# gmongaras/Stable-Diffusion-3-From-Scratch

Measured on AMD Instinct MI355X. Metric: train images/sec MMDiT-B 256^2 bf16, higher is better.
Workload: dtype bf16

## Files before the change

stable-diffusion-3-from-scratch_amd/csrc/rowops.hip:

```cpp
#include "qk_rows.h"
#include "fp8_quant.h"
#include "../../include/mmdit_hip_hd128.h"
#include "../../include/mmdit_hip_mxpad.h"

namespace {

constexpr float LN_EPS = 1e-5f;

__device__ __forceinline__ float bf16_round(float x) { return __builtin_bit_cast(float, pack_bf2(x, 0.f) << 16); }

template <int NITX, typename TO, typename TA, bool RES, bool MX = false, bool PAD = false>
__device__ __forceinline__ void ln_mod_fwd_body(int block, const float* __restrict__ x, const float* __restrict__ scale, const float* __restrict__ shift,
                                                int64_t ld_mod, int rows, int d, int rpb, TO* __restrict__ out,
                                                float* __restrict__ mean_o, float* __restrict__ rstd_o,
                                                const TA* __restrict__ acc, const float* __restrict__ gate, int64_t ld_gate, float* __restrict__ xo,
                                                unsigned char* __restrict__ mx_scales) {
  constexpr int NIT = NITX < 0 ? -NITX : NITX;
  constexpr bool EXACT = NITX < 0;
  const int lane = threadIdx.x & 63, row = block * 4 + (threadIdx.x >> 6);
  if (row >= rows) return;
  const int nch = d >> 2;
  const int b = row / rpb;
  const float* xr = x + (int64_t)row * d;
  float v[NIT][4];
  float s = 0.f;
#pragma unroll
  for (int it = 0; it < NIT; it++) {
    int ch = lane + 64 * it;
    if (EXACT || ch < nch) {
      ld4(xr + ch * 4, v[it]);
      if constexpr (RES) {
        float av[4], g[4];
        ld4(acc + (int64_t)row * d + ch * 4, av);
        ld4(gate + (int64_t)b * ld_gate + ch * 4, g);
#pragma unroll
        for (int e = 0; e < 4; e++) v[it][e] = v[it][e] + g[e] * av[e];
        __builtin_nontemporal_store(f32x4{v[it][0], v[it][1], v[it][2], v[it][3]}, (f32x4*)(xo + (int64_t)row * d + ch * 4));
      }
      s += v[it][0] + v[it][1] + v[it][2] + v[it][3];
    }
    else { v[it][0] = v[it][1] = v[it][2] = v[it][3] = 0.f; }
  }
  const float mean = wave_sum(s) / d;
  float q = 0.f;
#pragma unroll
  for (int it = 0; it < NIT; it++) {
    int ch = lane + 64 * it;
    if (EXACT || ch < nch) {
#pragma unroll
      for (int e = 0; e < 4; e++) { float c = v[it][e] - mean; q += c * c; }
    }
  }
  const float rstd = rsqrtf(wave_sum(q) / d + LN_EPS);
  if (lane == 0) { mean_o[row] = mean; rstd_o[row] = rstd; }
  const float* sc = scale + (int64_t)b * ld_mod;
  const float* sh = shift + (int64_t)b * ld_mod;
  TO* orow = out + (int64_t)row * d;
  const int ldo = PAD ? d + 64 : d;
  if constexpr (PAD) {
    if (lane < 4) *(uint4*)((unsigned char*)out + (int64_t)row * ldo + d + lane * 16) = make_uint4(0u, 0u, 0u, 0u);
    if (lane < 2) mx_scales[mx_scale_index(row, (d >> 5) + lane, rows)] = 0;
  }
#pragma unroll
  for (int it = 0; it < NIT; it++) {
    int ch = lane + 64 * it;
    if (EXACT || ch < nch) {
      float a[4], h[4], o[4];
      ld4(sc + ch * 4, a); ld4(sh + ch * 4, h);
#pragma unroll
      for (int e = 0; e < 4; e++) o[e] = (v[it][e] - mean) * rstd * (1.f + a[e]) + h[e];
      if constexpr (MX) {
#pragma unroll
        for (int e = 0; e < 4; e++) o[e] = bf16_round(o[e]);
        float amax = fmaxf(fmaxf(fabsf(o[0]), fabsf(o[1])), fmaxf(fabsf(o[2]), fabsf(o[3])));
        amax = fmaxf(amax, __shfl_xor(amax, 1, 64));
        amax = fmaxf(amax, __shfl_xor(amax, 2, 64));
        amax = fmaxf(amax, __shfl_xor(amax, 4, 64));
        float inv;
        const int ex = mx_exponent(amax, inv);
        *(unsigned*)((unsigned char*)out + (int64_t)row * ldo + ch * 4) = mx_pack4(o, inv);
        if ((lane & 7) == 0) mx_scales[mx_scale_index(row, ch >> 3, rows)] = (unsigned char)(ex + 127);
      } else {
        st4(orow + ch * 4, o);
      }
    }
  }
}

struct LnFwdProb {
  const float* x; const float* scale; const float* shift; int64_t ld_mod; int rows, rpb; void* out; float* mean; float* rstd;
  const void* acc; const float* gate; int64_t ld_gate; float* xo; unsigned char* mx_scales;
};
template <int NIT, typename TO, typename TA, bool RES, bool MX = false, bool PAD = false>
__global__ __launch_bounds__(256) void ln_mod_fwd_kernel(LnFwdProb p0, LnFwdProb p1, int nblk0, int d) {
  const bool first = (int)blockIdx.x < nblk0;
  const LnFwdProb& p = first ? p0 : p1;
  ln_mod_fwd_body<NIT, TO, TA, RES, MX, PAD>(first ? (int)blockIdx.x : (int)blockIdx.x - nblk0, p.x, p.scale, p.shift, p.ld_mod, p.rows, d, p.rpb, (TO*)p.out, p.mean, p.rstd,
                                        (const TA*)p.acc, p.gate, p.ld_gate, p.xo, p.mx_scales);
}

template <typename TA>
__global__ __launch_bounds__(256) void gate_residual_fwd_kernel(const float* __restrict__ x, const TA* __restrict__ acc, const float* __restrict__ gate, int64_t ld_gate,
                                                                int rows, int d, int rpb, float* __restrict__ out) {
  const int nch = d >> 2;
  for (int64_t i = (int64_t)blockIdx.x * 256 + threadIdx.x; i < (int64_t)rows * nch; i += (int64_t)gridDim.x * 256) {
    const int row = (int)(i / nch), ch = (int)(i - (int64_t)row * nch);
    float xv[4], av[4], g[4];
    ld4(x + (int64_t)row * d + ch * 4, xv);
    ld4(acc + (int64_t)row * d + ch * 4, av);
    ld4(gate + (int64_t)(row / rpb) * ld_gate + ch * 4, g);
#pragma unroll
    for (int e = 0; e < 4; e++) xv[e] = xv[e] + g[e] * av[e];
    st4(out + (int64_t)row * d + ch * 4, xv);
  }
}

#ifndef MMDIT_LN_BWD_RCH
#define MMDIT_LN_BWD_RCH 16
#endif
constexpr int LN_BWD_RCH = MMDIT_LN_BWD_RCH;
template <int NITX, typename TG, typename TA, bool GATED>
__device__ __forceinline__ void ln_mod_bwd_body(int block, const TG* __restrict__ dout, const float* __restrict__ x, const float* __restrict__ mean_i,
                                                const float* __restrict__ rstd_i, const float* __restrict__ scale, int64_t ld_mod,
                                                const float* __restrict__ dres, int d, int rpb, int nchunk,
                                                float* __restrict__ dx, float* __restrict__ dscale, float* __restrict__ dshift, int64_t ld_dmod,
                                                const TA* __restrict__ acc, const float* __restrict__ gate, int64_t ld_gate, TA* __restrict__ dacc,
                                                float* __restrict__ dgate, int64_t ld_dgate, float* __restrict__ dbias, int64_t ld_dbias, int rch = LN_BWD_RCH) {
  constexpr int NIT = NITX < 0 ? -NITX : NITX;
  constexpr bool EXACT = NITX < 0;
  const int lane = threadIdx.x & 63, wave = threadIdx.x >> 6;
  const int b = block / nchunk, chunk = block % nchunk;
  const int nch = d >> 2;
  const float* sc = scale + (int64_t)b * ld_mod;
  __shared__ float s_a1[NIT * 256], s_gt[GATED ? NIT * 256 : 4];
  for (int c = threadIdx.x; c < NIT * 256; c += 256) {
    s_a1[c] = c < d ? sc[c] + 1.f : 0.f;
    if constexpr (GATED) s_gt[c] = c < d ? gate[(int64_t)b * ld_gate + c] : 0.f;
  }
  __syncthreads();
  float ds[NIT][4], dh[NIT][4];
  float sg[GATED ? NIT : 1][4], sb[GATED ? NIT : 1][4];
#pragma unroll
  for (int it = 0; it < NIT; it++) {
#pragma unroll
    for (int e = 0; e < 4; e++) { ds[it][e] = 0.f; dh[it][e] = 0.f; }
    if constexpr (GATED) {
#pragma unroll
      for (int e = 0; e < 4; e++) { sg[it][e] = 0.f; sb[it][e] = 0.f; }
    }
  }
  const int rend = min(rpb, (chunk + 1) * rch);
  for (int rl = chunk * rch + wave; rl < rend; rl += 4) {
    const int64_t row = (int64_t)b * rpb + rl;
    const float mean = mean_i[row], rstd = rstd_i[row];
    float g[NIT][4], xh[NIT][4];
    float c1 = 0.f, c2 = 0.f;
    asm volatile("" ::: "memory");
#pragma unroll
    for (int it = 0; it < NIT; it++) {
      int ch = lane + 64 * it;
      if (EXACT || ch < nch) {
        float dy[4], xv[4], a1[4];
        ld4_nt(dout + row * d + ch * 4, dy);
        ld4_nt(x + row * d + ch * 4, xv);
        ld4(s_a1 + ch * 4, a1);
#pragma unroll
        for (int e = 0; e < 4; e++) {
          xh[it][e] = (xv[e] - mean) * rstd;
          g[it][e] = dy[e] * a1[e];
          c1 += g[it][e]; c2 += g[it][e] * xh[it][e];
          ds[it][e] += dy[e] * xh[it][e]; dh[it][e] += dy[e];
        }
      }
    }
    c1 = wave_sum(c1) / d; c2 = wave_sum(c2) / d;
#pragma unroll
    for (int it = 0; it < NIT; it++) {
      int ch = lane + 64 * it;
      if (EXACT || ch < nch) {
        float o[4];
        if (dres) ld4(dres + row * d + ch * 4, o); else { o[0] = o[1] = o[2] = o[3] = 0.f; }
#pragma unroll
        for (int e = 0; e < 4; e++) o[e] += rstd * (g[it][e] - c1 - xh[it][e] * c2);
        st4(dx + row * d + ch * 4, o);
        if constexpr (GATED) {
          float av[4], da[4], gt[4];
          ld4_nt(acc + row * d + ch * 4, av);
          ld4(s_gt + ch * 4, gt);
#pragma unroll
          for (int e = 0; e < 4; e++) { da[e] = o[e] * gt[e]; sg[it][e] += o[e] * av[e]; sb[it][e] += da[e]; }
          st4(dacc + row * d + ch * 4, da);
        }
      }
    }
  }
  if constexpr (NIT <= 6) {
    __shared__ float red[4][NIT * 256];
    auto flush = [&](const float (&v)[NIT][4], float* dst) {
#pragma unroll
      for (int it = 0; it < NIT; it++)
#pragma unroll
        for (int e = 0; e < 4; e++) red[wave][(it * 64 + lane) * 4 + e] = v[it][e];
      __syncthreads();
      for (int c = threadIdx.x; c < d; c += 256) atomicAdd(dst + c, red[0][c] + red[1][c] + red[2][c] + red[3][c]);
      __syncthreads();
    };
    flush(ds, dscale + (int64_t)b * ld_dmod);
    flush(dh, dshift + (int64_t)b * ld_dmod);
    if constexpr (GATED) {
      flush(sg, dgate + (int64_t)b * ld_dgate);
      if (dbias) flush(sb, dbias + (int64_t)b * ld_dbias);
    }
  } else {
    auto flush = [&](const float (&v)[NIT][4], float* dst) {
#pragma unroll
      for (int it = 0; it < NIT; it++) {
        int ch = lane + 64 * it;
        if (EXACT || ch < nch) {
#pragma unroll
          for (int e = 0; e < 4; e++) atomicAdd(dst + ch * 4 + e, v[it][e]);
        }
      }
    };
    flush(ds, dscale + (int64_t)b * ld_dmod);
    flush(dh, dshift + (int64_t)b * ld_dmod);
    if constexpr (GATED) {
      flush(sg, dgate + (int64_t)b * ld_dgate);
      if (dbias) flush(sb, dbias + (int64_t)b * ld_dbias);
    }
  }
}

struct LnBwdProb {
  const void* dout; const float* x; const float* mean; const float* rstd; const float* scale; int64_t ld_mod; const float* dres; int rpb, nchunk;
  float* dx; float* dscale; float* dshift; int64_t ld_dmod;
  const void* acc; const float* gate; int64_t ld_gate; void* dacc; float* dgate; int64_t ld_dgate; float* dbias; int64_t ld_dbias;
};
template <int NIT, typename TG, typename TA, bool GATED>
__global__ __launch_bounds__(256) void ln_mod_bwd_kernel(LnBwdProb p0, LnBwdProb p1, int nblk0, int d, int rch) {
  const bool first = (int)blockIdx.x < nblk0;
  const LnBwdProb& p = first ? p0 : p1;
  ln_mod_bwd_body<NIT, TG, TA, GATED>(first ? (int)blockIdx.x : (int)blockIdx.x - nblk0, (const TG*)p.dout, p.x, p.mean, p.rstd, p.scale, p.ld_mod, p.dres, d, p.rpb, p.nchunk,
                                      p.dx, p.dscale, p.dshift, p.ld_dmod, (const TA*)p.acc, p.gate, p.ld_gate, (TA*)p.dacc, p.dgate, p.ld_dgate, p.dbias, p.ld_dbias, rch);
}

template <int NITX, typename TI, typename TO>
__global__ __launch_bounds__(256) void text_rms_fwd_kernel(const TI* __restrict__ x, const float* __restrict__ w, const float* __restrict__ sp,
                                                           int rows, int cnt, int tokens, int off, int d, TO* __restrict__ out) {
  constexpr int NIT = NITX < 0 ? -NITX : NITX;
  constexpr bool EXACT = NITX < 0;
  const int lane = threadIdx.x & 63, m = blockIdx.x * 4 + (threadIdx.x >> 6);
// ... 593 lines not shown
    float* dst = which == 0 ? dgate + (int64_t)b * ld_dgate : (dbias ? dbias + (int64_t)b * ld_dbias : nullptr);
    if (!dst) break;
#pragma unroll
    for (int e = 0; e < 8; e++) sbuf[ty * 256 + tx * 8 + e] = which == 0 ? sgate[e] : sb[e];
    __syncthreads();
    if (col < d) {
      float s = 0.f;
#pragma unroll
      for (int r = 0; r < 8; r++) s += sbuf[r * 256 + threadIdx.x];
      atomicAdd(dst + col, s);
    }
    __syncthreads();
  }
}

template <typename T>
__global__ __launch_bounds__(256) void colsum_kernel(const T* __restrict__ x, int rows, int cols, int64_t ld, float* __restrict__ out, int rch) {
  __shared__ float sbuf[1024];
  const int tx = threadIdx.x & 127, ty = threadIdx.x >> 7;
  const int c = blockIdx.x * 1024 + tx * 8;
  float s[8];
#pragma unroll
  for (int e = 0; e < 8; e++) s[e] = 0.f;
  if (c < cols) {
    const int rend = min(rows, (int)(blockIdx.y + 1) * rch);
#pragma unroll 4
    for (int r = blockIdx.y * rch + ty; r < rend; r += 2) {
      float v[8];
      ld8(x + r * ld + c, v);
#pragma unroll
      for (int e = 0; e < 8; e++) s[e] += v[e];
    }
  }
  colsum_flush(s, sbuf, out, c, cols);
}

template <typename TG, typename TO>
__global__ __launch_bounds__(256) void silu_bwd_kernel(const TG* __restrict__ dy, const float* __restrict__ pre, TO* __restrict__ dpre, int rpg, int cols, float* __restrict__ dbias) {
  __shared__ float sb[4][64];
  const int cl = threadIdx.x & 63, rl = threadIdx.x >> 6;
  const int c = blockIdx.x * 64 + cl;
  const int r0 = blockIdx.y * rpg;
  float s = 0.f;
  if (c < cols) {
#pragma unroll 4
    for (int r = r0 + rl; r < r0 + rpg; r += 4) {
      const int64_t i = (int64_t)r * cols + c;
      const float p = pre[i], sig = sigmoid_f(p);
      const float g = io<TG>::ld(dy + i) * sig * (1.f + p * (1.f - sig));
      io<TO>::st(dpre + i, g);
      s += g;
    }
  }
  sb[rl][cl] = s;
  __syncthreads();
  if (rl == 0 && c < cols && dbias) dbias[(int64_t)blockIdx.y * cols + c] += sb[0][cl] + sb[1][cl] + sb[2][cl] + sb[3][cl];
}

template <typename TI, typename TO>
__global__ void cast_kernel(const TI* __restrict__ src, TO* __restrict__ dst, int64_t n) {
  const int64_t n8 = n >> 3;
  for (int64_t i = (int64_t)blockIdx.x * blockDim.x + threadIdx.x; i < n8; i += (int64_t)gridDim.x * blockDim.x) {
    float v[8];
    ld8(src + i * 8, v);
    st8(dst + i * 8, v);
  }
  if (blockIdx.x == 0 && threadIdx.x < (n & 7)) io<TO>::st(dst + n8 * 8 + threadIdx.x, io<TI>::ld(src + n8 * 8 + threadIdx.x));
}

template <typename TI, typename TO, bool TO_TOKENS>
__global__ void patch_kernel(const TI* __restrict__ src, TO* __restrict__ dst, int batch, int ch, int H, int W) {
  const int W2 = W >> 1, H2 = H >> 1;
  const int64_t total = (int64_t)batch * ch * H * W2;
  for (int64_t g = (int64_t)blockIdx.x * blockDim.x + threadIdx.x; g < total; g += (int64_t)gridDim.x * blockDim.x) {
    const int j = (int)(g % W2); int64_t r = g / W2;
    const int y = (int)(r % H); r /= H;
    const int c = (int)(r % ch); const int64_t b = r / ch;
    const int64_t img_off = ((b * ch + c) * H + y) * W + 2 * j;
    const int64_t tok_off = ((b * H2 + (y >> 1)) * W2 + j) * (int64_t)(ch * 4) + c * 4 + (y & 1) * 2;
    if (TO_TOKENS) { io<TO>::st(dst + tok_off, io<TI>::ld(src + img_off)); io<TO>::st(dst + tok_off + 1, io<TI>::ld(src + img_off + 1)); }
    else { io<TO>::st(dst + img_off, io<TI>::ld(src + tok_off)); io<TO>::st(dst + img_off + 1, io<TI>::ld(src + tok_off + 1)); }
  }
}

template <typename TO>
__global__ void time_embed_fwd_kernel(const float* __restrict__ t, const float* __restrict__ ts, const float* __restrict__ denom, int batch, int dim, TO* __restrict__ out) {
  const int i = blockIdx.x * blockDim.x + threadIdx.x, b = blockIdx.y;
  if (i >= dim) return;
  const float tau = t[b] * ts[0];
  const int half = dim >> 1;
  const float v = i < half ? sinf(tau / denom[2 * i]) : cosf(tau / denom[2 * (i - half) + 1]);
  io<TO>::st(out + (int64_t)b * dim + i, v);
}

template <typename TG>
__global__ __launch_bounds__(256) void time_embed_bwd_kernel(const TG* __restrict__ dout, const float* __restrict__ t, const float* __restrict__ ts,
                                                             const float* __restrict__ denom, int batch, int dim, float* __restrict__ dts) {
  __shared__ float red[4];
  const int b = blockIdx.x;
  const float tau = t[b] * ts[0];
  const int half = dim >> 1;
  float s = 0.f;
  for (int i = threadIdx.x; i < dim; i += 256) {
    const float g = io<TG>::ld(dout + (int64_t)b * dim + i);
    if (i < half) { const float dn = denom[2 * i]; s += g * cosf(tau / dn) / dn; }
    else { const float dn = denom[2 * (i - half) + 1]; s -= g * sinf(tau / dn) / dn; }
  }
  s = wave_sum(s);
  if ((threadIdx.x & 63) == 0) red[threadIdx.x >> 6] = s;
  __syncthreads();
  if (threadIdx.x == 0) atomicAdd(dts, (red[0] + red[1] + red[2] + red[3]) * t[b]);
}

inline int nit_for(int d) { return (d / 4 + 63) / 64; }
inline int grid_cap(int64_t n, int bs) { int64_t g = (n + bs - 1) / bs; return (int)(g < 1 ? 1 : g > 4096 ? 4096 : g); }

}

#define NIT_CASE(n, ...)                                                        \
  { if (d == (n) * 256) { constexpr int NIT = -(n); __VA_ARGS__; } else { constexpr int NIT = (n); __VA_ARGS__; } }
#define NIT_SWITCH(nit, ...)                                    \
  do {                                                          \
    if (nit <= 1) NIT_CASE(1, __VA_ARGS__)                      \
    else if (nit <= 2) NIT_CASE(2, __VA_ARGS__)                 \
    else if (nit <= 3) NIT_CASE(3, __VA_ARGS__)                 \
    else if (nit <= 4) NIT_CASE(4, __VA_ARGS__)                 \
    else if (nit <= 6) NIT_CASE(6, __VA_ARGS__)                 \
    else if (nit <= 9) NIT_CASE(9, __VA_ARGS__)                 \
    else if (nit <= 12) NIT_CASE(12, __VA_ARGS__)               \
    else NIT_CASE(16, __VA_ARGS__)                              \
  } while (0)

#define LN_FWD_NIT (NIT < 0 ? -NIT : NIT)

extern "C" int mmdit_abi_version(void) { return MMDIT_ABI_VERSION; }
extern "C" int mmdit_struct_size(int which) {
  switch (which) {
    case 0: return (int)sizeof(mmdit_gemm_args);
    case 1: return (int)sizeof(mmdit_ln_fwd_problem);
    case 2: return (int)sizeof(mmdit_ln_bwd_problem);
    case 3: return (int)sizeof(mmdit_qk_problem);
    case 4: return (int)sizeof(mmdit_mlp_bwd_problem);
    case 5: return (int)sizeof(mmdit_adamw_tensor);
    case 6: return (int)sizeof(mmdit_cast_tensor);
    case 7: return (int)sizeof(mmdit_qk_epilogue);
    default: return -1;
  }
}
extern "C" const char* mmdit_build_arch(void) { return "gfx950"; }

static int ln_mod_fwd_launch(const mmdit_ln_fwd_problem* probs, int count, int d, int out_dtype, unsigned char* const* mx_scales, hipStream_t s, bool pad = false) {
  MMDIT_CHECK_ARG(probs && count >= 1 && count <= 2 && d > 0 && d % 4 == 0 && d <= 4096);
  const bool res = probs[0].acc != nullptr;
  LnFwdProb q[2] = {};
  int nb[2] = {0, 0};
  for (int i = 0; i < count; i++) {
    const mmdit_ln_fwd_problem* p = probs + i;
    MMDIT_CHECK_ARG((p->acc != nullptr) == res);
    MMDIT_CHECK_ARG(p->x && p->scale && p->shift && p->out && p->mean && p->rstd && p->rows > 0 && p->rows_per_batch > 0 && p->ld_mod % 4 == 0);
    if (res) MMDIT_CHECK_ARG(p->gate && p->x_out && p->ld_gate % 4 == 0);
    q[i] = LnFwdProb{p->x, p->scale, p->shift, p->ld_mod, p->rows, p->rows_per_batch, p->out, p->mean, p->rstd, p->acc, p->gate, p->ld_gate, p->x_out, mx_scales ? mx_scales[i] : nullptr};
    nb[i] = (p->rows + 3) / 4;
  }
  const int nit = nit_for(d);
  dim3 grid(nb[0] + nb[1]);
#define LNL(TO, TA, RES, ...) NIT_SWITCH(nit, hipLaunchKernelGGL((ln_mod_fwd_kernel<LN_FWD_NIT, TO, TA, RES, __VA_ARGS__>), grid, dim3(256), 0, s, q[0], q[1], nb[0], d))
  if (mx_scales && pad) { if (res) { LNL(unsigned char, bf16_t, true, true, true); } else { LNL(unsigned char, bf16_t, false, true, true); } }
  else if (mx_scales) { if (res) { LNL(unsigned char, bf16_t, true, true); } else { LNL(unsigned char, bf16_t, false, true); } }
  else if (out_dtype == MMDIT_BF16) { if (res) { LNL(bf16_t, bf16_t, true, false); } else { LNL(bf16_t, bf16_t, false, false); } }
  else if (out_dtype == MMDIT_F32) { if (res) { LNL(float, float, true, false); } else { LNL(float, float, false, false); } }
  else return MMDIT_ERR_DTYPE;
#undef LNL
  return mmdit_launch_status();
}

extern "C" int mmdit_ln_modulate_fwd(const mmdit_ln_fwd_problem* probs, int count, int d, int acc_dtype, int out_dtype, mmdit_stream_t stream) {
  MMDIT_CHECK_ARG(probs && count >= 1 && (!probs[0].acc || acc_dtype == out_dtype));
  return ln_mod_fwd_launch(probs, count, d, out_dtype, nullptr, (hipStream_t)stream);
}

extern "C" int mmdit_ln_modulate_fwd_mx(const float* x, const void* acc, int acc_dtype, const float* gate, int64_t ld_gate, float* x_out,
                                        const float* scale, const float* shift, int64_t ld_mod, int rows, int d, int rpb,
                                        void* q_fp8, void* scales_e8m0, float* mean, float* rstd, mmdit_stream_t stream) {
  MMDIT_CHECK_ARG(scales_e8m0 && d % 64 == 0 && (!acc || acc_dtype == MMDIT_BF16));
  const mmdit_ln_fwd_problem p = {x, acc, gate, ld_gate, x_out, scale, shift, ld_mod, rows, rpb, q_fp8, mean, rstd};
  unsigned char* const sc[1] = {(unsigned char*)scales_e8m0};
  return ln_mod_fwd_launch(&p, 1, d, MMDIT_FP8, sc, (hipStream_t)stream);
}

extern "C" int mmdit_ln_modulate_fwd_mx_pad(const mmdit_ln_fwd_problem* probs, int count, int d, int acc_dtype, void* scales_e8m0_0, void* scales_e8m0_1,
                                            mmdit_stream_t stream) {
  MMDIT_CHECK_ARG(probs && count >= 1 && count <= 2 && scales_e8m0_0 && (count == 1 || scales_e8m0_1));
  if (d <= 0 || d % 64 != 0) return MMDIT_ERR_SHAPE;
  for (int i = 0; i < count; i++)
    if (probs[i].rows > 0 && (int64_t)probs[i].rows * ((d + 127) / 128 * 128) / 16 > 0x7fffffffll) return MMDIT_ERR_SHAPE;
  MMDIT_CHECK_ARG(!probs[0].acc || acc_dtype == MMDIT_BF16);
  unsigned char* const sc[2] = {(unsigned char*)scales_e8m0_0, (unsigned char*)scales_e8m0_1};
  return ln_mod_fwd_launch(probs, count, d, MMDIT_FP8, sc, (hipStream_t)stream, d % 128 != 0);
}

extern "C" int mmdit_gate_residual_fwd(const float* x, const void* acc, int acc_dtype, const float* gate, int64_t ld_gate, int rows, int d, int rpb,
                                       float* out, mmdit_stream_t stream) {
  MMDIT_CHECK_ARG(x && acc && gate && out && rows > 0 && d > 0 && d % 4 == 0 && rpb > 0 && ld_gate % 4 == 0);
  hipStream_t s = (hipStream_t)stream;
  dim3 grid(grid_cap((int64_t)rows * (d / 4), 256));
  if (acc_dtype == MMDIT_BF16) hipLaunchKernelGGL((gate_residual_fwd_kernel<bf16_t>), grid, dim3(256), 0, s, x, (const bf16_t*)acc, gate, ld_gate, rows, d, rpb, out);
  else if (acc_dtype == MMDIT_F32) hipLaunchKernelGGL((gate_residual_fwd_kernel<float>), grid, dim3(256), 0, s, x, (const float*)acc, gate, ld_gate, rows, d, rpb, out);
  else return MMDIT_ERR_DTYPE;
  return mmdit_launch_status();
}

static int ln_bwd_one_round_rch(const mmdit_ln_bwd_problem* a, const mmdit_ln_bwd_problem* b, int d, int dout_dtype, bool gated) {
  auto wgs = [&](int r) { return (long)(a->rows / a->rows_per_batch) * ((a->rows_per_batch + r - 1) / r) + (long)(b->rows / b->rows_per_batch) * ((b->rows_per_batch + r - 1) / r); };
  const int nit_ = nit_for(d), nit_abs = nit_ < 0 ? -nit_ : nit_;
  int per_cu = nit_abs <= 3 ? 4 : nit_abs == 4 ? 3 : 2, cus = 256;
  {
    static int occ[64][17][2][2], cu_count[64];
    const int dev = mmdit_current_device(), ti = dout_dtype == MMDIT_BF16 ? 0 : 1, gi = gated ? 1 : 0, ni = nit_abs > 16 ? 16 : nit_abs;
    if (!cu_count[dev]) {
      int n = 0;
      cu_count[dev] = (hipDeviceGetAttribute(&n, hipDeviceAttributeMultiprocessorCount, dev) == hipSuccess && n > 0) ? n : 256;
    }
    cus = cu_count[dev];
    if (!occ[dev][ni][ti][gi]) {
      int nbq = 0;
      hipError_t e = hipErrorUnknown;
#define LNQ(T, G) NIT_SWITCH(nit_, e = hipOccupancyMaxActiveBlocksPerMultiprocessor(&nbq, (const void*)ln_mod_bwd_kernel<(NIT < 0 ? -NIT : NIT), T, T, G>, 256, 0))
      if (dout_dtype == MMDIT_BF16) { if (gated) { LNQ(bf16_t, true); } else { LNQ(bf16_t, false); } }
      else if (dout_dtype == MMDIT_F32) { if (gated) { LNQ(float, true); } else { LNQ(float, false); } }
#undef LNQ
      occ[dev][ni][ti][gi] = (e == hipSuccess && nbq > 0) ? nbq : 8;
    }
    per_cu = per_cu < occ[dev][ni][ti][gi] ? per_cu : occ[dev][ni][ti][gi];
  }
  const long slots = (long)cus * per_cu;
  if (wgs(LN_BWD_RCH) > slots && wgs(LN_BWD_RCH) <= 2 * slots)
    for (int r = LN_BWD_RCH + 4; r <= 64; r += 4)
      if (wgs(r) <= slots) return r;
  return LN_BWD_RCH;
}

extern "C" int mmdit_ln_modulate_bwd(const mmdit_ln_bwd_problem* probs, int count, int d, int dout_dtype, mmdit_stream_t stream) {
  MMDIT_CHECK_ARG(probs && count >= 1 && count <= 2 && d > 0 && d % 4 == 0 && d <= 4096);
  const bool gated = probs[0].acc != nullptr;
  for (int i = 0; i < count; i++) {
    const mmdit_ln_bwd_problem* p = probs + i;
    MMDIT_CHECK_ARG((p->acc != nullptr) == gated);
    MMDIT_CHECK_ARG(p->dout && p->x && p->mean && p->rstd && p->scale && p->dx && p->dscale && p->dshift && p->rows > 0 && p->rows_per_batch > 0 &&
                    p->rows % p->rows_per_batch == 0 && p->ld_mod % 4 == 0);
    if (gated) MMDIT_CHECK_ARG(p->gate && p->dacc && p->dgate && p->ld_gate % 4 == 0);
  }
  if (dout_dtype != MMDIT_BF16 && dout_dtype != MMDIT_F32) return MMDIT_ERR_DTYPE;
  const int rch = count == 2 ? ln_bwd_one_round_rch(probs, probs + 1, d, dout_dtype, gated) : LN_BWD_RCH;
  LnBwdProb q[2] = {};
  int nb[2] = {0, 0};
  for (int i = 0; i < count; i++) {
    const mmdit_ln_bwd_problem* p = probs + i;
    const int nchunk = (p->rows_per_batch + rch - 1) / rch;
    nb[i] = (p->rows / p->rows_per_batch) * nchunk;
    q[i] = LnBwdProb{p->dout, p->x, p->mean, p->rstd, p->scale, p->ld_mod, p->dres, p->rows_per_batch, nchunk, p->dx, p->dscale, p->dshift, p->ld_dmod,
                     p->acc, p->gate, p->ld_gate, p->dacc, p->dgate, p->ld_dgate, p->dbias, p->ld_dbias};
  }
  hipStream_t s = (hipStream_t)stream;
  const int nit = nit_for(d);
  dim3 grid(nb[0] + nb[1]);
#define LNL(T, G) NIT_SWITCH(nit, hipLaunchKernelGGL((ln_mod_bwd_kernel<(NIT < 0 ? -NIT : NIT), T, T, G>), grid, dim3(256), 0, s, q[0], q[1], nb[0], d, rch))
  if (dout_dtype == MMDIT_BF16) { if (gated) { LNL(bf16_t, true); } else { LNL(bf16_t, false); } }
  else { if (gated) { LNL(float, true); } else { LNL(float, false); } }
#undef LNL
  return mmdit_launch_status();
}

extern "C" int mmdit_text_rmsnorm_fwd(const void* x, int x_dtype, const float* w1, const float* w2, const float* s1, const float* s2,
                                      int batch, int tokens, int split, int d, void* out1, void* out2, int out_dtype, mmdit_stream_t stream) {
  MMDIT_CHECK_ARG(x && w1 && w2 && s1 && s2 && out1 && out2 && batch > 0 && split > 0 && split < tokens && d % 4 == 0 && d <= 4096);
  hipStream_t s = (hipStream_t)stream;
  const int nit = nit_for(d);
  for (int half = 0; half < 2; half++) {
    const int cnt = half ? tokens - split : split, off = half ? split : 0, rows = batch * cnt;
    const float* w = half ? w2 : w1; const float* sp = half ? s2 : s1; void* out = half ? out2 : out1;
    dim3 grid((rows + 3) / 4);
#define TRF(TI, TO) NIT_SWITCH(nit, hipLaunchKernelGGL((text_rms_fwd_kernel<LN_FWD_NIT, TI, TO>), grid, dim3(256), 0, s, (const TI*)x, w, sp, rows, cnt, tokens, off, d, (TO*)out))
    if (x_dtype == MMDIT_F32 && out_dtype == MMDIT_F32) { TRF(float, float); }
    else if (x_dtype == MMDIT_F32 && out_dtype == MMDIT_BF16) { TRF(float, bf16_t); }
    else if (x_dtype == MMDIT_BF16 && out_dtype == MMDIT_BF16) { TRF(bf16_t, bf16_t); }
    else if (x_dtype == MMDIT_BF16 && out_dtype == MMDIT_F32) { TRF(bf16_t, float); }
    else return MMDIT_ERR_DTYPE;
#undef TRF
  }
  return mmdit_launch_status();
}

extern "C" int mmdit_text_rmsnorm_bwd(const void* dout1, const void* dout2, int dout_dtype, const void* x, int x_dtype,
                                      const float* w1, const float* w2, const float* s1, const float* s2, int batch, int tokens, int split, int d,
                                      float* dw1, float* dw2, float* ds1, float* ds2, mmdit_stream_t stream) {
  MMDIT_CHECK_ARG(dout1 && dout2 && x && w1 && w2 && s1 && s2 && dw1 && dw2 && ds1 && ds2 && batch > 0 && split > 0 && split < tokens && d % 4 == 0 && d <= 4096);
  hipStream_t s = (hipStream_t)stream;
  const int nit = nit_for(d);
  TextRmsBwdHalf h[2];
  int maxrows = 0;
  for (int half = 0; half < 2; half++) {
    const int cnt = half ? tokens - split : split, rows = batch * cnt;
    h[half] = TextRmsBwdHalf{half ? dout2 : dout1, half ? w2 : w1, half ? s2 : s1, rows, cnt, half ? split : 0, half ? dw2 : dw1, half ? ds2 : ds1};
    maxrows = rows > maxrows ? rows : maxrows;
  }
  dim3 grid((maxrows + TRB_ROWS - 1) / TRB_ROWS, 2);
#define TRB(TI, TG) NIT_SWITCH(nit, hipLaunchKernelGGL((text_rms_bwd_kernel<NIT, TI, TG>), grid, dim3(512), 0, s, h[0], h[1], (const TI*)x, tokens, d))
  if (x_dtype == MMDIT_F32 && dout_dtype == MMDIT_F32) { TRB(float, float); }
  else if (x_dtype == MMDIT_F32 && dout_dtype == MMDIT_BF16) { TRB(float, bf16_t); }
  else if (x_dtype == MMDIT_BF16 && dout_dtype == MMDIT_BF16) { TRB(bf16_t, bf16_t); }
  else if (x_dtype == MMDIT_BF16 && dout_dtype == MMDIT_F32) { TRB(bf16_t, float); }
  else return MMDIT_ERR_DTYPE;
#undef TRB
  return mmdit_launch_status();
}

constexpr int QK_RL_MIN_ROWS = 2048;
static_assert(QK_RL_MIN_ROWS == MMDIT_QK_HD128_RL_MIN_ROWS && 1024 / (3 * 128 / 8) == MMDIT_QK_HD128_MAX_HEADS, "include/mmdit_hip_hd128.h documents this policy");
static int qk_rl(int row_threads, int min_rows) {
// ... 386 lines not shown
```

Baseline: 2321.

## Process row chunks per block in LN-modulate forward with LDS-cached modulation

Reworks the LayerNorm+modulate forward kernel so each block handles a chunk of up to 16 rows from a single batch instead of 4 rows. The per-batch scale (precomputed as 1+scale), shift and gate vectors are staged once in shared memory, and the next row's x/acc loads are software-prefetched while the current row is reduced. The aim is to cut redundant global loads of modulation vectors and hide load latency. The trade-off is fewer blocks (less parallelism), an added __syncthreads, and extra shared memory and registers.

After: 2324, median of 6. Within noise of the previous version (+0.1%).

```diff
diff --git a/stable-diffusion-3-from-scratch_amd/csrc/rowops.hip b/stable-diffusion-3-from-scratch_amd/csrc/rowops.hip
--- a/stable-diffusion-3-from-scratch_amd/csrc/rowops.hip
+++ b/stable-diffusion-3-from-scratch_amd/csrc/rowops.hip
@@ -7,96 +7,146 @@
 
 constexpr float LN_EPS = 1e-5f;
 
+template <typename T> struct raw4;
+template <> struct raw4<float> { typedef f32x4 type; };
+template <> struct raw4<bf16_t> { typedef u32x2 type; };
+template <bool NT, typename T>
+__device__ __forceinline__ typename raw4<T>::type ld4_raw(const T* p) {
+  typedef typename raw4<T>::type R;
+  if constexpr (NT) return __builtin_nontemporal_load((const R*)p);
+  else return *(const R*)p;
+}
+__device__ __forceinline__ void widen4(f32x4 a, float (&v)[4]) { asm volatile("" : "+v"(a)); v[0] = a[0]; v[1] = a[1]; v[2] = a[2]; v[3] = a[3]; }
+__device__ __forceinline__ void widen4(u32x2 a, float (&v)[4]) {
+  asm volatile("" : "+v"(a));
+  v[0] = __builtin_bit_cast(float, a[0] << 16); v[1] = __builtin_bit_cast(float, a[0] & 0xffff0000u);
+  v[2] = __builtin_bit_cast(float, a[1] << 16); v[3] = __builtin_bit_cast(float, a[1] & 0xffff0000u);
+}
+
+#ifndef MMDIT_LN_FWD_RCH
+#define MMDIT_LN_FWD_RCH 16
+#endif
+constexpr int LN_FWD_RCH = MMDIT_LN_FWD_RCH;
 __device__ __forceinline__ float bf16_round(float x) { return __builtin_bit_cast(float, pack_bf2(x, 0.f) << 16); }
 
 template <int NITX, typename TO, typename TA, bool RES, bool MX = false, bool PAD = false>
 __device__ __forceinline__ void ln_mod_fwd_body(int block, const float* __restrict__ x, const float* __restrict__ scale, const float* __restrict__ shift,
-                                                int64_t ld_mod, int rows, int d, int rpb, TO* __restrict__ out,
+                                                int64_t ld_mod, int rows, int d, int rpb, int nchunk, int rch, TO* __restrict__ out,
                                                 float* __restrict__ mean_o, float* __restrict__ rstd_o,
                                                 const TA* __restrict__ acc, const float* __restrict__ gate, int64_t ld_gate, float* __restrict__ xo,
                                                 unsigned char* __restrict__ mx_scales) {
   constexpr int NIT = NITX < 0 ? -NITX : NITX;
   constexpr bool EXACT = NITX < 0;
-  const int lane = threadIdx.x & 63, row = block * 4 + (threadIdx.x >> 6);
-  if (row >= rows) return;
+  const int lane = threadIdx.x & 63, wave = __builtin_amdgcn_readfirstlane(threadIdx.x >> 6);
+  const int b = block / nchunk, chunk = block - b * nchunk;
   const int nch = d >> 2;
-  const int b = row / rpb;
-  const float* xr = x + (int64_t)row * d;
-  float v[NIT][4];
-  float s = 0.f;
-#pragma unroll
-  for (int it = 0; it < NIT; it++) {
-    int ch = lane + 64 * it;
-    if (EXACT || ch < nch) {
-      ld4(xr + ch * 4, v[it]);
-      if constexpr (RES) {
-        float av[4], g[4];
-        ld4(acc + (int64_t)row * d + ch * 4, av);
-        ld4(gate + (int64_t)b * ld_gate + ch * 4, g);
-#pragma unroll
-        for (int e = 0; e < 4; e++) v[it][e] = v[it][e] + g[e] * av[e];
-        __builtin_nontemporal_store(f32x4{v[it][0], v[it][1], v[it][2], v[it][3]}, (f32x4*)(xo + (int64_t)row * d + ch * 4));
-      }
-      s += v[it][0] + v[it][1] + v[it][2] + v[it][3];
-    }
-    else { v[it][0] = v[it][1] = v[it][2] = v[it][3] = 0.f; }
-  }
-  const float mean = wave_sum(s) / d;
-  float q = 0.f;
-#pragma unroll
-  for (int it = 0; it < NIT; it++) {
-    int ch = lane + 64 * it;
-    if (EXACT || ch < nch) {
-#pragma unroll
-      for (int e = 0; e < 4; e++) { float c = v[it][e] - mean; q += c * c; }
-    }
-  }
-  const float rstd = rsqrtf(wave_sum(q) / d + LN_EPS);
-  if (lane == 0) { mean_o[row] = mean; rstd_o[row] = rstd; }
-  const float* sc = scale + (int64_t)b * ld_mod;
-  const float* sh = shift + (int64_t)b * ld_mod;
-  TO* orow = out + (int64_t)row * d;
+  const int row0 = b * rpb;
+  const int rend = min(min(rpb, rows - row0), (chunk + 1) * rch);
+  int rl = chunk * rch + wave;
+  typename raw4<float>::type xr[NIT];
+  typename raw4<TA>::type ar[RES ? NIT : 1];
+  auto load_row = [&](int r) {
+    const int64_t base = (int64_t)(row0 + r) * d;
+#pragma unroll
+    for (int it = 0; it < NIT; it++) {
+      const int cl = EXACT ? lane + 64 * it : min(lane + 64 * it, nch - 1);
+      xr[it] = ld4_raw<false>(x + base + cl * 4);
+      if constexpr (RES) ar[it] = ld4_raw<false>(acc + base + cl * 4);
+    }
+  };
+  if (rl < rend) load_row(rl);
+  __shared__ float s_a1[NIT * 256], s_sh[NIT * 256], s_gt[RES ? NIT * 256 : 4];
+  for (int c = threadIdx.x; c < NIT * 256; c += 256) {
+    s_a1[c] = c < d ? 1.f + scale[(int64_t)b * ld_mod + c] : 0.f;
+    s_sh[c] = c < d ? shift[(int64_t)b * ld_mod + c] : 0.f;
+    if constexpr (RES) s_gt[c] = c < d ? gate[(int64_t)b * ld_gate + c] : 0.f;
+  }
+  __syncthreads();
   const int ldo = PAD ? d + 64 : d;
-  if constexpr (PAD) {
-    if (lane < 4) *(uint4*)((unsigned char*)out + (int64_t)row * ldo + d + lane * 16) = make_uint4(0u, 0u, 0u, 0u);
-    if (lane < 2) mx_scales[mx_scale_index(row, (d >> 5) + lane, rows)] = 0;
-  }
-#pragma unroll
-  for (int it = 0; it < NIT; it++) {
-    int ch = lane + 64 * it;
-    if (EXACT || ch < nch) {
-      float a[4], h[4], o[4];
-      ld4(sc + ch * 4, a); ld4(sh + ch * 4, h);
-#pragma unroll
-      for (int e = 0; e < 4; e++) o[e] = (v[it][e] - mean) * rstd * (1.f + a[e]) + h[e];
-      if constexpr (MX) {
-#pragma unroll
-        for (int e = 0; e < 4; e++) o[e] = bf16_round(o[e]);
-        float amax = fmaxf(fmaxf(fabsf(o[0]), fabsf(o[1])), fmaxf(fabsf(o[2]), fabsf(o[3])));
-        amax = fmaxf(amax, __shfl_xor(amax, 1, 64));
-        amax = fmaxf(amax, __shfl_xor(amax, 2, 64));
-        amax = fmaxf(amax, __shfl_xor(amax, 4, 64));
-        float inv;
-        const int ex = mx_exponent(amax, inv);
-        *(unsigned*)((unsigned char*)out + (int64_t)row * ldo + ch * 4) = mx_pack4(o, inv);
-        if ((lane & 7) == 0) mx_scales[mx_scale_index(row, ch >> 3, rows)] = (unsigned char)(ex + 127);
-      } else {
-        st4(orow + ch * 4, o);
+  for (; rl < rend; rl += 4) {
+    const int row = row0 + rl;
+    asm volatile("" ::: "memory");
+    float v[NIT][4];
+    float s = 0.f;
+#pragma unroll
+    for (int it = 0; it < NIT; it++) {
+      int ch = lane + 64 * it;
+      if (EXACT || ch < nch) {
+        widen4(xr[it], v[it]);
+        if constexpr (RES) {
+          float av[4], g[4];
+          widen4(ar[it], av);
+          ld4(s_gt + ch * 4, g);
+#pragma unroll
+          for (int e = 0; e < 4; e++) v[it][e] = v[it][e] + g[e] * av[e];
+        }
+        s += v[it][0] + v[it][1] + v[it][2] + v[it][3];
+      }
+      else { v[it][0] = v[it][1] = v[it][2] = v[it][3] = 0.f; }
+    }
+    if constexpr (RES) {
+#pragma unroll
+      for (int it = 0; it < NIT; it++) {
+        int ch = lane + 64 * it;
+        if (EXACT || ch < nch)
+          __builtin_nontemporal_store(f32x4{v[it][0], v[it][1], v[it][2], v[it][3]}, (f32x4*)(xo + (int64_t)row * d + ch * 4));
+      }
+    }
+    if (rl + 4 < rend) load_row(rl + 4);
+    const float mean = wave_sum(s) / d;
+    float q = 0.f;
+#pragma unroll
+    for (int it = 0; it < NIT; it++) {
+      int ch = lane + 64 * it;
+      if (EXACT || ch < nch) {
+#pragma unroll
+        for (int e = 0; e < 4; e++) { float c = v[it][e] - mean; q += c * c; }
+      }
+    }
+    const float rstd = rsqrtf(wave_sum(q) / d + LN_EPS);
+    if (lane == 0) { mean_o[row] = mean; rstd_o[row] = rstd; }
+    TO* orow = out + (int64_t)row * d;
+    if constexpr (PAD) {
+      if (lane < 4) *(uint4*)((unsigned char*)out + (int64_t)row * ldo + d + lane * 16) = make_uint4(0u, 0u, 0u, 0u);
+      if (lane < 2) mx_scales[mx_scale_index(row, (d >> 5) + lane, rows)] = 0;
+    }
+#pragma unroll
+    for (int it = 0; it < NIT; it++) {
+      int ch = lane + 64 * it;
+      if (EXACT || ch < nch) {
+        float a1[4], h[4], o[4];
+        ld4(s_a1 + ch * 4, a1); ld4(s_sh + ch * 4, h);
+#pragma unroll
+        for (int e = 0; e < 4; e++) o[e] = (v[it][e] - mean) * rstd * a1[e] + h[e];
+        if constexpr (MX) {
+#pragma unroll
+          for (int e = 0; e < 4; e++) o[e] = bf16_round(o[e]);
+          float amax = fmaxf(fmaxf(fabsf(o[0]), fabsf(o[1])), fmaxf(fabsf(o[2]), fabsf(o[3])));
+          amax = fmaxf(amax, __shfl_xor(amax, 1, 64));
+          amax = fmaxf(amax, __shfl_xor(amax, 2, 64));
+          amax = fmaxf(amax, __shfl_xor(amax, 4, 64));
+          float inv;
+          const int ex = mx_exponent(amax, inv);
+          *(unsigned*)((unsigned char*)out + (int64_t)row * ldo + ch * 4) = mx_pack4(o, inv);
+          if ((lane & 7) == 0) mx_scales[mx_scale_index(row, ch >> 3, rows)] = (unsigned char)(ex + 127);
+        } else {
+          st4(orow + ch * 4, o);
+        }
       }
     }
   }
 }
 
 struct LnFwdProb {
-  const float* x; const float* scale; const float* shift; int64_t ld_mod; int rows, rpb; void* out; float* mean; float* rstd;
+  const float* x; const float* scale; const float* shift; int64_t ld_mod; int rows, rpb, nchunk; void* out; float* mean; float* rstd;
   const void* acc; const float* gate; int64_t ld_gate; float* xo; unsigned char* mx_scales;
 };
 template <int NIT, typename TO, typename TA, bool RES, bool MX = false, bool PAD = false>
-__global__ __launch_bounds__(256) void ln_mod_fwd_kernel(LnFwdProb p0, LnFwdProb p1, int nblk0, int d) {
+__global__ __launch_bounds__(256) void ln_mod_fwd_kernel(LnFwdProb p0, LnFwdProb p1, int nblk0, int d, int rch) {
   const bool first = (int)blockIdx.x < nblk0;
   const LnFwdProb& p = first ? p0 : p1;
-  ln_mod_fwd_body<NIT, TO, TA, RES, MX, PAD>(first ? (int)blockIdx.x : (int)blockIdx.x - nblk0, p.x, p.scale, p.shift, p.ld_mod, p.rows, d, p.rpb, (TO*)p.out, p.mean, p.rstd,
-                                        (const TA*)p.acc, p.gate, p.ld_gate, p.xo, p.mx_scales);
+  ln_mod_fwd_body<NIT, TO, TA, RES, MX, PAD>(first ? (int)blockIdx.x : (int)blockIdx.x - nblk0, p.x, p.scale, p.shift, p.ld_mod, p.rows, d, p.rpb, p.nchunk, rch, (TO*)p.out, p.mean,
+                                             p.rstd, (const TA*)p.acc, p.gate, p.ld_gate, p.xo, p.mx_scales);
 }
 
 template <typename TA>
@@ -996,6 +1046,7 @@
 static int ln_mod_fwd_launch(const mmdit_ln_fwd_problem* probs, int count, int d, int out_dtype, unsigned char* const* mx_scales, hipStream_t s, bool pad = false) {
   MMDIT_CHECK_ARG(probs && count >= 1 && count <= 2 && d > 0 && d % 4 == 0 && d <= 4096);
   const bool res = probs[0].acc != nullptr;
+  const int rch = LN_FWD_RCH;
   LnFwdProb q[2] = {};
   int nb[2] = {0, 0};
   for (int i = 0; i < count; i++) {
@@ -1003,12 +1054,13 @@
     MMDIT_CHECK_ARG((p->acc != nullptr) == res);
     MMDIT_CHECK_ARG(p->x && p->scale && p->shift && p->out && p->mean && p->rstd && p->rows > 0 && p->rows_per_batch > 0 && p->ld_mod % 4 == 0);
     if (res) MMDIT_CHECK_ARG(p->gate && p->x_out && p->ld_gate % 4 == 0);
-    q[i] = LnFwdProb{p->x, p->scale, p->shift, p->ld_mod, p->rows, p->rows_per_batch, p->out, p->mean, p->rstd, p->acc, p->gate, p->ld_gate, p->x_out, mx_scales ? mx_scales[i] : nullptr};
-    nb[i] = (p->rows + 3) / 4;
+    const int nchunk = ((p->rows < p->rows_per_batch ? p->rows : p->rows_per_batch) + rch - 1) / rch;
+    q[i] = LnFwdProb{p->x, p->scale, p->shift, p->ld_mod, p->rows, p->rows_per_batch, nchunk, p->out, p->mean, p->rstd, p->acc, p->gate, p->ld_gate, p->x_out, mx_scales ? mx_scales[i] : nullptr};
+    nb[i] = (int)(((int64_t)p->rows + p->rows_per_batch - 1) / p->rows_per_batch) * nchunk;
   }
   const int nit = nit_for(d);
   dim3 grid(nb[0] + nb[1]);
-#define LNL(TO, TA, RES, ...) NIT_SWITCH(nit, hipLaunchKernelGGL((ln_mod_fwd_kernel<LN_FWD_NIT, TO, TA, RES, __VA_ARGS__>), grid, dim3(256), 0, s, q[0], q[1], nb[0], d))
+#define LNL(TO, TA, RES, ...) NIT_SWITCH(nit, hipLaunchKernelGGL((ln_mod_fwd_kernel<LN_FWD_NIT, TO, TA, RES, __VA_ARGS__>), grid, dim3(256), 0, s, q[0], q[1], nb[0], d, rch))
   if (mx_scales && pad) { if (res) { LNL(unsigned char, bf16_t, true, true, true); } else { LNL(unsigned char, bf16_t, false, true, true); } }
   else if (mx_scales) { if (res) { LNL(unsigned char, bf16_t, true, true); } else { LNL(unsigned char, bf16_t, false, true); } }
   else if (out_dtype == MMDIT_BF16) { if (res) { LNL(bf16_t, bf16_t, true, false); } else { LNL(bf16_t, bf16_t, false, false); } }
```
